# kernel-matrix-benchmarks/kernel-matrix-benchmarks

Hardware: AMD Instinct MI355X
Metric: point-pair interactions/s (N*M/s) + max |err| vs scipy, D=3 Gaussian (higher is better)
Workload: dtype f32

## Files before the change

### kernel_matrix_benchmarks_amd/csrc/kmvp_api.hip

```cpp
#include "kmvp_ctx.hpp"

namespace kmvp {

Rccl g_rccl;

namespace {
thread_local std::string g_create_error;
}

int fail(kmvp_ctx* c, int code, const std::string& msg) {
  if (c) c->err = msg;
  else g_create_error = msg;
  return code;
}
const char* create_error() { return g_create_error.c_str(); }

int ensure(kmvp_ctx* c, DevBuf& b, size_t bytes) {
  if (bytes <= b.cap && b.p) return KMVP_OK;
  if (b.p) {
    HIP_TRY(c, hipFree(b.p));
    b.p = nullptr;
    b.cap = 0;
  }
  if (bytes == 0) bytes = 16;
// ... 264 lines not shown
  if (r1 != ncclSuccess || r2 != ncclSuccess || count != world || user_rank != rank) {
    g_rccl.CommDestroy(c->comm);
    c->comm = nullptr;
    c->comm_count = 1;
    c->rank = 0;
    c->world = 1;
    return fail(c, KMVP_E_COMM, "RCCL communicator mismatch: asked for rank " + std::to_string(rank) + " of " +
                                    std::to_string(world) + " on device " + std::to_string(c->device) + ", RCCL reports rank " +
                                    std::to_string(user_rank) + " of " + std::to_string(count) + " on device " +
                                    std::to_string(dev));
  }
  c->comm_count = count;
  c->rank = rank;
  c->world = world;
  return KMVP_OK;
}

int kmvp_comm_init_host(kmvp_ctx* c, kmvp_host_allreduce_fn fn, void* user, int rank, int world) {
  if (!c || !fn || world < 1 || rank < 0 || rank >= world) return fail(c, KMVP_E_INVALID, "bad communicator arguments");
  if (c->comm) {
    g_rccl.CommDestroy(c->comm);
    c->comm = nullptr;
  }
  c->host_xchg = fn;
  c->host_user = user;
  c->comm_count = world;
  c->rank = rank;
  c->world = world;
  return KMVP_OK;
}

int kmvp_comm_world(const kmvp_ctx* c) { return (c && c->exchanges()) ? c->comm_count : 1; }
int kmvp_comm_rank(const kmvp_ctx* c) { return (c && c->exchanges()) ? c->rank : 0; }

int kmvp_set_option(kmvp_ctx* c, const char* key, int64_t value) {
  if (!c || !key) return KMVP_E_INVALID;
  const std::string k(key);
  if (k == "feed") {
    if (value < -1 || value > 1) return fail(c, KMVP_E_INVALID, "feed must be -1 (auto), 0 or 1");
    c->opt_feed = (int)value;
  } else if (k == "targets_per_lane") {
    if (value != 0 && value != 1 && value != 2 && value != 4 && value != 8)
      return fail(c, KMVP_E_INVALID, "targets_per_lane must be 0 (auto), 1, 2, 4 or 8");
    c->opt_T = (int)value;
  } else if (k == "segments") {
    if (value < 0 || value > 65535) return fail(c, KMVP_E_INVALID, "segments out of range");
    c->opt_segments = (int)value;
  } else if (k == "fast_sqdists") {
    if (value < -1 || value > 4) return fail(c, KMVP_E_INVALID, "fast_sqdists must be -1 (auto), 0, 1, 2, 3 or 4");
    c->opt_fast = (int)value;
  } else if (k == "cellmm_shape") {
    if (value < -1 || value > 1) return fail(c, KMVP_E_INVALID, "cellmm_shape must be -1 (by size), 0 (32x32x16) or 1 (16x16x32)");
    c->opt_cellmm_shape = (int)value;
  } else if (k == "cell_fused") {
    if (value < -1 || value > 1) return fail(c, KMVP_E_INVALID, "cell_fused must be -1 (automatic), 0 (two launches) or 1 (one launch where it applies)");
    c->opt_cell_fused = (int)value;
  } else if (k == "mfma_variant") {
    if (value != -1 && value != 0 && value != 1 && value != 4 && value != 5)
      return fail(c, KMVP_E_INVALID, "mfma_variant must be -1 (by kernel), 0, 1, 4 or 5");
    c->opt_mfma_variant = (int)value;
  } else if (k == "same_points_global") {
    c->opt_same_global = value != 0;
  } else if (k == "partial_shard") {
    c->opt_partial = value != 0;
  } else if (k == "fast_tiles") {
    if (value != 0 && value != 1 && value != 2 && value != 4 && value != 8)
      return fail(c, KMVP_E_INVALID, "fast_tiles must be 0 (auto), 1, 2, 4 or 8");
    c->opt_fast_tiles = (int)value;
  } else if (k == "chunk") {
    if (value < 8 || value > (1 << 24)) return fail(c, KMVP_E_INVALID, "chunk out of range");
    c->opt_chunk = (int)value;
  } else {
    return fail(c, KMVP_E_INVALID, "unknown option " + k);
  }
  return KMVP_OK;
}

int64_t kmvp_device_bytes(const kmvp_ctx* c) {
  if (!c) return 0;
  size_t t = 0;
  for (const DevBuf* b : {&c->y_raw, &c->x_raw, &c->b_raw, &c->xs, &c->rec, &c->x_scaled,
                          &c->y_scaled, &c->part, &c->partd, &c->aux, &c->sortbuf, &c->perm, &c->sums, &c->out, &c->scratch, &c->sdiag, &c->xchg, &c->kexp, &c->kshift, &c->xchgk, &c->kflag,
                    &c->sk_xs_x, &c->sk_rec_y, &c->sk_xs_y, &c->sk_rec_x, &c->sk_state,
                          &c->cell_tperm, &c->cell_sperm, &c->cell_tgrp, &c->cell_sgrp, &c->cell_slot, &c->cell_tmeta, &c->cell_sums, &c->cell_skey, &c->cell_scentre, &c->cell_scale})
    t += b->cap;
  return (int64_t)t;
}
double kmvp_last_kernel_ms(const kmvp_ctx* c) { return c ? c->last_kernel_ms : 0.0; }
double kmvp_last_total_ms(const kmvp_ctx* c) { return c ? c->last_total_ms : 0.0; }
double kmvp_last_allreduce_ms(const kmvp_ctx* c) { return c ? c->last_allreduce_ms : 0.0; }
const char* kmvp_last_kernel_name(const kmvp_ctx* c) { return c ? c->last_kernel_name : ""; }
const char* kmvp_last_dispatch_note(const kmvp_ctx* c) { return c ? c->note.c_str() : ""; }

}
```

### kernel_matrix_benchmarks_amd/csrc/kmvp_cellmm.hpp

```cpp
#pragma once
#include <hip/hip_runtime.h>
#include <stdint.h>

#include "kmvp_cell.hpp"

namespace kmvp {

#ifndef CMM_BF16
#define CMM_BF16 0
#endif
#if CMM_BF16
typedef __bf16 cmm_half;
#else
typedef _Float16 cmm_half;
#endif
typedef cmm_half f16x8 __attribute__((ext_vector_type(8)));
typedef cmm_half f16x2 __attribute__((ext_vector_type(2)));

constexpr int CMM_STAGE_TILES = 12;
constexpr int CMM_STAGE_BYTES = 8192;
constexpr int CMM_E_OFF = 0;
constexpr int CMM_B_OFF = CMM_STAGE_TILES * CELL_TILE * 16;
constexpr int CMM_HDR_OFF = CMM_B_OFF + CMM_STAGE_TILES * CELL_TILE * 4;
static_assert(CMM_HDR_OFF + CMM_STAGE_TILES * 16 <= CMM_STAGE_BYTES, "stage image too small");
constexpr float CMM_TARGET_SCALE = 64.f;
constexpr int CMM_MAX_WLOG2 = 8;

struct CellmmArgs {
  const float* xd;
  const float* tmeta;
  const unsigned char* img;
  const float* scale;
  double* part;
  int64_t n_slots;
  int64_t tile_base;
  int64_t m_stages;
  int64_t seg_stages;
  int segments;
  int tile_blocks;
};

typedef int i32x4 __attribute__((ext_vector_type(4)));

__device__ __forceinline__ f16x2 cellmm_pk(float a, float b) {
#if CMM_BF16
  f16x2 r;
  r[0] = (cmm_half)a;
  r[1] = (cmm_half)b;
  return r;
#else
  return __builtin_bit_cast(f16x2, __builtin_amdgcn_cvt_pkrtz(a, b));
#endif
}

__device__ __forceinline__ f16x8 cellmm_target_operand(const f32x4 d, int h) {
  float s[3], sh[3], sm[3];
#pragma unroll
  for (int c = 0; c < 3; ++c) {
    s[c] = d[c] * CMM_TARGET_SCALE;
    sh[c] = (float)(cmm_half)s[c];
    sm[c] = s[c] - sh[c];
  }
  const float q = CMM_TARGET_SCALE;
  float lo[8], hi[8];
  lo[0] = sh[0]; lo[1] = sh[1]; lo[2] = sh[0]; lo[3] = sh[1]; lo[4] = sm[0]; lo[5] = sm[1];
  lo[6] = d[0] * d[0] * (0.5f * q);
  lo[7] = d[1] * d[1] * (0.5f * q);
  hi[0] = sh[2]; hi[1] = d[0] * d[2] * q; hi[2] = sh[2]; hi[3] = d[0] * d[2] * q; hi[4] = sm[2];
  hi[5] = d[1] * d[2] * q;
  hi[6] = d[2] * d[2] * (0.5f * q);
  hi[7] = d[0] * d[1] * q;
  f16x8 out;
#pragma unroll
  for (int j = 0; j < 8; ++j) out[j] = (cmm_half)(h ? hi[j] : lo[j]);
  return out;
}

typedef float f32x2 __attribute__((ext_vector_type(2)));

template <int CTRL, int ROWMASK>
__device__ __forceinline__ float cellmm_dpp(float v) {
  return __int_as_float(__builtin_amdgcn_update_dpp(0, __float_as_int(v), CTRL, ROWMASK, 0xf, false));
}
__device__ __forceinline__ float cellmm_half_sum(float v) {
  v += cellmm_dpp<0x111, 0xf>(v);
  v += cellmm_dpp<0x112, 0xf>(v);
  v += cellmm_dpp<0x114, 0xf>(v);
  v += cellmm_dpp<0x118, 0xf>(v);
  v += cellmm_dpp<0x142, 0xa>(v);
  return __int_as_float(__builtin_amdgcn_readlane(__float_as_int(v), 31));
}
__device__ __forceinline__ float cellmm_cross_half_add(float v) {
// ... 144 lines not shown
      const float u1 = a14[0] * wb, u2 = a14[1] * wb;
      const f16x2 R0 = cellmm_pk(u1, u2);
      const float c1 = (float)R0[0], c2 = (float)R0[1];
      const f16x2 R1 = cellmm_pk(u1 - c1, u2 - c2);
      const f16x2 R3 = cellmm_pk(a14[2] * wb, a14[3] * wb);
      const f16x2 R2 = cellmm_pk(c1, a5 * wb);
      i32x4 yw;
      yw[0] = __builtin_bit_cast(int, R0);
      yw[1] = __builtin_bit_cast(int, R1);
      yw[2] = __builtin_bit_cast(int, R2);
      yw[3] = __builtin_bit_cast(int, R3);
      const f16x8 ya = __builtin_bit_cast(f16x8, yw);
#pragma unroll
      for (int tt = 0; tt < TT; ++tt) {
#if CMM_BF16
        acc[tt] = __builtin_amdgcn_mfma_f32_32x32x16_bf16(ya, xb[tt], acc[tt], 0, 0, 0);
#else
        acc[tt] = __builtin_amdgcn_mfma_f32_32x32x16_f16(ya, xb[tt], acc[tt], 0, 0, 0);
#endif
      }
    }
    if (s + 1 < s_end) commit(buf ^ 1);
    __syncthreads();
  }
  if (key_s >= 0) fold();

  const double inv = (double)a.scale[1];
#pragma unroll
  for (int tt = 0; tt < TT; ++tt)
    if (h == 0) a.part[(int64_t)seg * a.n_slots + (tile0 + tt - a.tile_base) * CELL_TILE + r] = outd[tt] * inv;
}


__device__ __forceinline__ float cellmm16_fold4(float a, float b, float c, float d) {
  const auto p = __builtin_amdgcn_permlane16_swap(__float_as_uint(a), __float_as_uint(b), false, false);
  const float w0 = __uint_as_float(p[0]) + __uint_as_float(p[1]);
  const auto q = __builtin_amdgcn_permlane16_swap(__float_as_uint(c), __float_as_uint(d), false, false);
  const float w1 = __uint_as_float(q[0]) + __uint_as_float(q[1]);
  const auto r = __builtin_amdgcn_permlane32_swap(__float_as_uint(w0), __float_as_uint(w1), false, false);
  return __uint_as_float(r[0]) + __uint_as_float(r[1]);
}
__device__ __forceinline__ float cellmm16_sources_sum(float v) {
  v += cellmm_dpp<0x111, 0xf>(v);
  v += cellmm_dpp<0x112, 0xf>(v);
  v += cellmm_dpp<0x114, 0xf>(v);
  v += cellmm_dpp<0x118, 0xf>(v);
  return __int_as_float(__builtin_amdgcn_readlane(__float_as_int(v), 15)) +
         __int_as_float(__builtin_amdgcn_readlane(__float_as_int(v), 47));
}

#ifndef CMM16_NOFOLD
#define CMM16_NOFOLD 0
#endif

template <int TT>
__device__ __forceinline__ void cellmm16_body(const CellmmArgs& a, int bid, unsigned char (*lds)[CMM_STAGE_BYTES]) {
  static_assert(!CMM_BF16, "f16 operands only");
  constexpr int SB = CMM_STAGE_BYTES;
  constexpr int PIECES = SB / (16 * BLOCK_THREADS);
  constexpr float LOG2E = 1.4426950408889634f;
  constexpr int HT = 2 * TT;
  constexpr int NG = (HT + 3) / 4;

  int tb, seg;
  block_to_work(bid, a.segments, a.tile_blocks, tb, seg);
  const int lane = threadIdx.x & 63;
  const int wave = threadIdx.x >> 6;
  const int cc = lane & 15;
  const int kg = lane >> 4;
  const int h = kg & 1;
  const int rs = 16 * (kg >> 1) + cc;
  const int64_t tile0 = a.tile_base + ((int64_t)tb * WAVES_PER_BLOCK + wave) * TT;

  float cT[3];
  f16x8 xb[HT];
#pragma unroll
  for (int u = 0; u < HT; ++u) {
    const f32x4 v = *reinterpret_cast<const f32x4*>(a.xd + ((tile0 + (u >> 1)) * CELL_TILE + 16 * (u & 1) + cc) * 4);
    xb[u] = cellmm_target_operand(v, h);
  }
  {
    const f32x4 m = *reinterpret_cast<const f32x4*>(a.tmeta + tile0 * 4);
#pragma unroll
    for (int c = 0; c < 3; ++c) cT[c] = __int_as_float(__builtin_amdgcn_readfirstlane(__float_as_int(m[c])));
  }
  float dl[NG][3], U[NG], vprev[NG];
  double outd[NG];
#pragma unroll
  for (int g = 0; g < NG; ++g) {
    const int u = 4 * g + kg < HT ? 4 * g + kg : HT - 1;
    const f32x4 v = *reinterpret_cast<const f32x4*>(a.xd + ((tile0 + (u >> 1)) * CELL_TILE + 16 * (u & 1) + cc) * 4);
#pragma unroll
    for (int c = 0; c < 3; ++c) dl[g][c] = v[c];
    U[g] = 0.f;
    vprev[g] = 0.f;
    outd[g] = 0.0;
  }

  f32x4 acc[HT];
#pragma unroll
  for (int u = 0; u < HT; ++u)
#pragma unroll
    for (int k = 0; k < 4; ++k) acc[u][k] = 0.f;

  const int64_t s_begin = (int64_t)seg * a.seg_stages;
  int64_t s_end = s_begin + a.seg_stages;
  if (s_end > a.m_stages) s_end = a.m_stages;

  f32x4 pre[PIECES];
  auto fetch = [&](int64_t s) {
    const unsigned char* src = a.img + s * SB;
#pragma unroll
    for (int p = 0; p < PIECES; ++p)
      pre[p] = *reinterpret_cast<const f32x4*>(src + (p * BLOCK_THREADS + (int)threadIdx.x) * 16);
  };
  auto commit = [&](int buf) {
#pragma unroll
    for (int p = 0; p < PIECES; ++p)
      *reinterpret_cast<f32x4*>(&lds[buf][(p * BLOCK_THREADS + (int)threadIdx.x) * 16]) = pre[p];
  };
  if (s_begin < s_end) {
    fetch(s_begin);
    commit(0);
  }
  __syncthreads();

  int key_s = -2;
  float S0 = 0.f, S0c = 0.f;
  float D1[3] = {0.f, 0.f, 0.f};

  auto fold = [&]() {
#if CMM16_NOFOLD
    asm volatile("" ::"v"(S0), "v"(S0c));
#else
    const float s0 = cellmm16_sources_sum(S0) * CMM_TARGET_SCALE;
    float x[4 * NG];
#pragma unroll
    for (int u = 0; u < 4 * NG; ++u) x[u] = u < HT ? (acc[u][0] + acc[u][1]) + (acc[u][2] + acc[u][3]) : 0.f;
#pragma unroll
    for (int g = 0; g < NG; ++g) {
      const float v = cellmm16_fold4(x[4 * g], x[4 * g + 1], x[4 * g + 2], x[4 * g + 3]);
      outd[g] += (double)(U[g] * ((v - vprev[g]) + s0));
      vprev[g] = v;
    }
#endif
    S0 = 0.f;
    S0c = 0.f;
  };
  auto new_cell = [&](const f32x4 cs, int ks) {
    if (key_s >= 0) fold();
    key_s = ks;
#pragma unroll
    for (int c = 0; c < 3; ++c) D1[c] = (cT[c] - cs[c]) * LOG2E;
#if !CMM16_NOFOLD
#pragma unroll
    for (int g = 0; g < NG; ++g) {
      float s2 = 0.f;
#pragma unroll
      for (int c = 0; c < 3; ++c) {
        const float df = dl[g][c] + (cT[c] - cs[c]);
        s2 = fmaf(df, df, s2);
      }
      U[g] = kexp2(s2 * -LOG2E);
    }
#endif
  };

  for (int64_t s = s_begin; s < s_end; ++s) {
    const int buf = (int)((s - s_begin) & 1);
    if (s + 1 < s_end) fetch(s + 1);
    const unsigned char* base = &lds[buf][0];
    const unsigned char* p_ef = base + CMM_E_OFF + rs * 16;
    const unsigned char* p_b = base + CMM_B_OFF + rs * 4;
    const f32x4* hdr = reinterpret_cast<const f32x4*>(base + CMM_HDR_OFF);
    const int keys = lane < CMM_STAGE_TILES ? __float_as_int(hdr[lane < CMM_STAGE_TILES ? lane : 0][3]) : -1;
#pragma unroll 1
    for (int q = 0; q < CMM_STAGE_TILES; ++q) {
      const int ks = __builtin_amdgcn_readlane(keys, q);
      if (ks < 0) break;
      if (ks != key_s) new_cell(hdr[q], ks);
      const f32x4 ef = *reinterpret_cast<const f32x4*>(p_ef);
      const float bq = *reinterpret_cast<const float*>(p_b);
      p_ef += CELL_TILE * 16;
      p_b += CELL_TILE * 4;
      const float m0 = h ? ef[2] : ef[0];
      const float m1 = h ? ef[0] : ef[1];
      const float m2 = h ? ef[2] : 1.f;
      const f32x4 a14 = f32x4{m0, m1 * m2, m0 * m0, m1 * ef[1]};
      const float a5 = ef[1] * m2;
      const float arg = fmaf(ef[0], D1[0], fmaf(ef[1], D1[1], fmaf(ef[2], D1[2], ef[3])));
      const float wb = kexp2(arg) * bq;
      {
        const float yk = wb - S0c;
        const float tk = S0 + yk;
        S0c = (tk - S0) - yk;
        S0 = tk;
      }
      const float u1 = a14[0] * wb, u2 = a14[1] * wb;
      const f16x2 R0 = cellmm_pk(u1, u2);
      const float c1 = (float)R0[0], c2 = (float)R0[1];
      const f16x2 R1 = cellmm_pk(u1 - c1, u2 - c2);
      const f16x2 R3 = cellmm_pk(a14[2] * wb, a14[3] * wb);
      const f16x2 R2 = cellmm_pk(c1, a5 * wb);
      i32x4 yw;
      yw[0] = __builtin_bit_cast(int, R0);
      yw[1] = __builtin_bit_cast(int, R1);
      yw[2] = __builtin_bit_cast(int, R2);
      yw[3] = __builtin_bit_cast(int, R3);
      const f16x8 ya = __builtin_bit_cast(f16x8, yw);
#pragma unroll
      for (int u = 0; u < HT; ++u) acc[u] = __builtin_amdgcn_mfma_f32_16x16x32_f16(ya, xb[u], acc[u], 0, 0, 0);
    }
    if (s + 1 < s_end) commit(buf ^ 1);
    __syncthreads();
  }
  if (key_s >= 0) fold();
#if CMM16_NOFOLD
#pragma unroll
  for (int u = 0; u < HT; ++u) asm volatile("" ::"v"(acc[u][0]), "v"(acc[u][1]), "v"(acc[u][2]), "v"(acc[u][3]));
#endif

  const double inv = (double)a.scale[1];
#pragma unroll
  for (int g = 0; g < NG; ++g)
    if (4 * g + kg < HT)
      a.part[(int64_t)seg * a.n_slots + (tile0 + 2 * g + (kg >> 1) - a.tile_base) * CELL_TILE + 16 * h + cc] = outd[g] * inv;
}

template <int TT>
__global__ void __launch_bounds__(BLOCK_THREADS) __attribute__((amdgpu_waves_per_eu(TT >= 8 ? 2 : 1)))
cellmm16_kernel(const CellmmArgs a, const CellmmArgs rest, const int main_grid) {
  __shared__ __attribute__((aligned(16))) unsigned char lds[2][CMM_STAGE_BYTES];
  if constexpr (TT > CELL_REST_TT) {
    const FusedCellWork w = fused_cell_work((int64_t)blockIdx.x, (int64_t)main_grid);
    if (w.list) {
      cellmm16_body<CELL_REST_TT>(rest, (int)w.local, lds);
      return;
    }
  }
  cellmm16_body<TT>(a, (int)blockIdx.x, lds);
}

hipError_t launch_cellmm_gaussian(int TT, int shape, const CellmmArgs& args, dim3 grid, hipStream_t stream, const char** kernel_name);
hipError_t launch_cellmm16_fused(int TT, const CellmmArgs& main, const CellmmArgs& rest, int64_t main_grid, int64_t rest_grid,
                                 hipStream_t stream, const char** kernel_name);

}
```

### kernel_matrix_benchmarks_amd/csrc/kmvp_ctx.hpp

```cpp
#pragma once
#include <dlfcn.h>
#include <hip/hip_runtime.h>
#include <rccl/rccl.h>
#include <stdint.h>
#include <stdlib.h>
#include <string.h>

#include <algorithm>
#include <cmath>
#include <string>
#include <vector>

#include "../../include/kmvp.h"
#include "kmvp_internal.hpp"

namespace kmvp {

enum : int { LAYOUT_LOWD = 0, LAYOUT_FAST = 1, LAYOUT_MFMA = 2, LAYOUT_CFAST = 3, LAYOUT_CELL = 4, LAYOUT_CELL64 = 5, LAYOUT_CELLMM = 6, LAYOUT_FASTMM = 7, LAYOUT_CFASTMM = 8 };

struct DevBuf {
  void* p = nullptr;
  size_t cap = 0;
};

// ... 50 lines not shown
      error = "librccl lacks an expected symbol";
      return false;
    }
    return true;
  }
};extern Rccl g_rccl;

}

struct kmvp_ctx {
  using DevBuf = kmvp::DevBuf;
  int device = 0;
  hipStream_t stream = nullptr;
  hipEvent_t ev[5] = {nullptr, nullptr, nullptr, nullptr, nullptr};
  std::string err;

  int dtype = -1;
  int D = 0, E = 0;
  int64_t M = 0, N = 0, j_offset = 0, m_total = 0;
  bool same_points = false;
  bool have_points = false, have_signal = false, density = false;
  bool async_product = false;
  bool diag_on = false;
  int64_t diag_n = 0;
  double diag_ridge = 0.0, diag_min = 0.0;

  DevBuf y_raw, x_raw, b_raw;
  DevBuf xs, rec;
  DevBuf partd;
  DevBuf aux;
  DevBuf sortbuf, perm;
  DevBuf x_scaled, y_scaled;
  DevBuf cell_tperm, cell_sperm, cell_tgrp, cell_sgrp, cell_slot, cell_tmeta, cell_sums, cell_skey, cell_scentre, cell_scale;
  DevBuf part, sums, out;
  DevBuf xchg;
  DevBuf kexp, kshift, xchgk;
  DevBuf kflag;
  DevBuf scratch;
  DevBuf sdiag;
  DevBuf sk_xs_x, sk_rec_y, sk_xs_y, sk_rec_x, sk_state;
  uint64_t sk_points_ver = 0;
  uint64_t points_ver = 0, signal_ver = 0;
  int packed_layout = -1;
  int packed_kernel = -1, packed_sig = -1, packed_T = -1;
  uint64_t packed_points_ver = 0, packed_signal_ver = 0;
  int gen_kernel = -1;
  uint64_t gen_points_ver = 0;
  int64_t out_n = 0;
  int out_e = 0;

  int opt_feed = -1, opt_T = 0, opt_segments = 0, opt_chunk = 512;
  int opt_fast = -1, opt_fast_tiles = 0;
  int opt_cellmm_shape = -1;
  int opt_cell_fused = -1;
  int opt_mfma_variant = -1;
  int opt_same_global = 0;
  int opt_partial = 0;
  uint64_t perm_ver = 0;
  uint64_t cell_ver = 0;
  int cell_state = 0;
  int cell_tt = 0, cell_tt_req = 0;
  float cell_lo[3] = {0.f, 0.f, 0.f}, cell_hh[3] = {1.f, 1.f, 1.f};
  int cell_g[3] = {1, 1, 1};
  int64_t cell_n_tiles = 0, cell_m_tiles = 0;
  int64_t cell_n_main = 0, cell_n_rest = 0;
  float cloud_radius2 = INFINITY;
  uint64_t centre_ver = 0;

  ncclComm_t comm = nullptr;
  int rank = 0, world = 1;
  kmvp_host_allreduce_fn host_xchg = nullptr;
  void* host_user = nullptr;
  std::vector<double> host_buf;
  bool exchanges() const { return comm != nullptr || host_xchg != nullptr; }

  int comm_count = 1;
  float last_kernel_ms = 0.f, last_total_ms = 0.f, last_allreduce_ms = 0.f;
  const char* last_kernel_name = "";
  std::string note;
};

namespace kmvp {

int fail(kmvp_ctx* c, int code, const std::string& msg);
const char* create_error();

#define HIP_TRY(c, expr)                                                                     \
  do {                                                                                       \
    hipError_t e_ = (expr);                                                                  \
    if (e_ != hipSuccess)                                                                    \
      return kmvp::fail((c), e_ == hipErrorOutOfMemory ? KMVP_E_NOMEM : KMVP_E_DEVICE,       \
                        std::string(#expr) + ": " + hipGetErrorString(e_));                  \
  } while (0)

inline size_t elem_size(int dtype) { return dtype == KMVP_F64 ? 8 : 4; }
inline unsigned blocks_for(int64_t n, int threads = 256) { return (unsigned)((n + threads - 1) / threads); }

int ensure(kmvp_ctx* c, DevBuf& b, size_t bytes);
void release(DevBuf& b);

int run_product(kmvp_ctx* c, int kernel, bool normalise);
int measure_clouds(kmvp_ctx* c, int dtype, int64_t M, int64_t N, int D);
int prepare_points(kmvp_ctx* c, int kernel);
int run_gradient(kmvp_ctx* c, int kernel);
int run_logsumexp(kmvp_ctx* c, int kernel);
int run_logsumexp_grad(kmvp_ctx* c, int kernel);

int cg_solve(kmvp_ctx* c, int kernel, const void* a_host, int E, double rtol, int maxit, double* out_b,
             int* iters, double* resid);
int minres_solve(kmvp_ctx* c, int kernel, const void* a_host, int E, double rtol, int maxit,
                 double* out_b, int* iters, double* resid);

int sinkhorn_solve(kmvp_ctx* c, int kernel, const double* log_a, const double* log_b, double tol, int maxit, double* u,
                   double* v, int* iters, double* err);

}
```

### kernel_matrix_benchmarks_amd/csrc/kmvp_plan.hpp

```cpp
#pragma once
#include <algorithm>
#include <cstdint>
#include <vector>

namespace kmvp {

constexpr int WAVES_PER_BLOCK = 4;
constexpr int CELL_TILE = 32;
constexpr int CELL_REST_TT = 2;
constexpr int STAGED_TILE = 32;
constexpr int64_t SMALL_PROBLEM_TARGETS = 32768;
constexpr int SEG_SPLIT_FROM = 16;
constexpr int64_t MAX_GRID = 0x7fffffff;

inline int64_t round_up(int64_t v, int64_t q) { return (v + q - 1) / q * q; }
inline bool small_problem(int64_t N) { return N < SMALL_PROBLEM_TARGETS; }


struct SegmentRule {
  int64_t stage_bytes;
  int cols;
  int64_t min_seg = 1;
  bool small = false;
  int64_t l2_seg_bytes = 2 << 20;
// ... 145 lines not shown
  int64_t grid(int r) const { return blocks[r] * segments[r]; }
  size_t region_offset(int cols, int r) const { return r ? (size_t)segments[0] * cols * slots[0] : 0; }
  size_t part_doubles(int cols) const { return ((size_t)segments[0] * slots[0] + (size_t)segments[1] * slots[1]) * cols; }
};

inline CellSplit cell_split(int64_t N, int64_t m_tiles, int64_t n_main, int64_t n_rest, int tt, int opt_segments,
                            int stage_tiles, SegmentRule main) {
  CellSplit s;
  main.small = small_problem(N);
  if (main.small) main.min_seg = 1;
  s.m_stages = (m_tiles + stage_tiles - 1) / stage_tiles;
  s.n_slots = (n_main + n_rest) * CELL_TILE;
  s.blocks[0] = n_main / (tt * WAVES_PER_BLOCK);
  s.blocks[1] = n_rest / (CELL_REST_TT * WAVES_PER_BLOCK);
  s.slots[0] = n_main * CELL_TILE;
  s.slots[1] = n_rest * CELL_TILE;
  s.segments[0] = stage_segments(opt_segments, std::max<int64_t>(1, s.blocks[0]), s.m_stages, s.n_slots, main);
  s.seg_stages[0] = (s.m_stages + s.segments[0] - 1) / s.segments[0];
  s.segments[1] = 0;
  s.seg_stages[1] = 1;
  if (s.blocks[1] > 0) {
    SegmentRule rest = main;
    rest.min_seg = 1;
    rest.target_blocks = 1536;
    const int seg = choose_segments(opt_segments, s.blocks[1], s.m_stages, s.n_slots, rest);
    s.seg_stages[1] = (s.m_stages + seg - 1) / seg;
    s.segments[1] = (int)((s.m_stages + s.seg_stages[1] - 1) / s.seg_stages[1]);
  }
  return s;
}


struct FusedCellWork {
  int list;
  int64_t local;
};
constexpr FusedCellWork fused_cell_work(int64_t bid, int64_t main_grid) {
  return bid < main_grid ? FusedCellWork{0, bid} : FusedCellWork{1, bid - main_grid};
}

struct FusedCellGrid {
  bool fused;
  int64_t main_grid, rest_grid, total;
};
inline FusedCellGrid fused_cell_grid(const CellSplit& s, int tt, int opt_fused) {
  FusedCellGrid g;
  g.main_grid = s.grid(0);
  g.rest_grid = s.grid(1);
  g.total = g.main_grid + g.rest_grid;
  g.fused = opt_fused != 0 && tt > CELL_REST_TT && s.blocks[1] > 0 && g.total <= MAX_GRID;
  return g;
}

}
```

### kernel_matrix_benchmarks_amd/csrc/kmvp_product.hip

```cpp
#include "kmvp_ctx.hpp"
#include <vector>
#include "kmvp_cell_pack.hpp"
#include "kmvp_cell64_pack.hpp"
#include "kmvp_cellmm_pack.hpp"
#include "kmvp_cfast_pack.hpp"
#include "kmvp_fast_pack.hpp"
#include "kmvp_fastmm_pack.hpp"
#include "kmvp_cfastmm_pack.hpp"
#include "kmvp_mfma_pack.hpp"

namespace kmvp {
namespace {

template <typename real>
hipError_t launch_lowd(int kernel, int D, int E, int sig, LowdTuning tune,
                       const LowdArgs<real>& args, dim3 grid, hipStream_t s, const char** name);
template <>
hipError_t launch_lowd<float>(int kernel, int D, int E, int sig, LowdTuning tune,
                              const LowdArgs<float>& args, dim3 grid, hipStream_t s,
                              const char** name) {
  switch (kernel) {
    case K_GAUSSIAN: return launch_lowd_gaussian_f32(D, E, sig, tune, args, grid, s, name);
    case K_ABSEXP: return launch_lowd_absexp_f32(D, E, sig, tune, args, grid, s, name);
    case K_INVDIST: return launch_lowd_invdist_f32(D, E, sig, tune, args, grid, s, name);
// ... 1208 lines not shown
    }
  }
  return true;
}
void cell_store_grid(kmvp_ctx* c, const CellGrid& grid) {
  for (int a = 0; a < 3; ++a) {
    c->cell_lo[a] = grid.lo[a];
    c->cell_g[a] = grid.g[a];
    c->cell_hh[a] = grid.h[a];
  }
}
void cell_load_grid(const kmvp_ctx* c, CellGrid& grid) {
  for (int a = 0; a < 3; ++a) {
    grid.lo[a] = c->cell_lo[a];
    grid.g[a] = c->cell_g[a];
    grid.h[a] = c->cell_hh[a];
    grid.inv_h[a] = 1.f / c->cell_hh[a];
  }
}

inline double cell_ps_per_tile(int TT) { return TT >= 8 ? CMM_PS_PER_TILE_MAIN : (TT >= 4 ? CMM_PS_PER_TILE_TT4 : CMM_PS_PER_TILE_REST); }

int cell_prepare(kmvp_ctx* c, int TT) {
  if (c->cell_ver == c->points_ver && c->cell_state != 0 && (c->cell_state < 0 || c->cell_tt_req == TT)) return KMVP_OK;
  c->cell_tt_req = TT;
  c->cell_ver = c->points_ver;
  c->cell_state = -1;
  const int D = c->D;
  if (D > CELL_MAX_D || !(c->cloud_radius2 < INFINITY) || c->N > 0x3fffffff || c->M > 0x3fffffff) return KMVP_OK;
  float aux[FAST_AUX_FLOATS];
  HIP_TRY(c, hipMemcpyAsync(aux, c->aux.p, sizeof(aux), hipMemcpyDeviceToHost, c->stream));
  HIP_TRY(c, hipStreamSynchronize(c->stream));
  CellGrid grid;
  if (!cell_make_grid(aux, D, (float)(std::sqrt(2.f * CELL_T_MAX / (float)D)), grid)) return KMVP_OK;
  int rc;
  std::vector<unsigned> keys;
  if ((rc = cell_sort(c, c->y_raw.p, c->M, grid, c->cell_sperm, keys))) return rc;
  const TileList sources = cell_tiles(keys.data(), c->M);
  if ((rc = upload_tiles(c, sources, c->cell_sgrp))) return rc;
  c->cell_m_tiles = (int64_t)sources.size();
  if (!c->same_points && (rc = cell_sort(c, c->x_raw.p, c->N, grid, c->cell_tperm, keys))) return rc;
  if (TT == 0) {
    double best = INFINITY;
    for (int t : {8, 4, 2}) {
      int64_t nm, nr;
      cell_split_count(keys.data(), (int64_t)keys.size(), t, &nm, &nr);
      const double cost = cell_ps_per_tile(t) * (double)nm + cell_ps_per_tile(2) * (double)nr;
      if (cost < best) {
        best = cost;
        TT = t;
      }
    }
  }
  if ((rc = upload_tiles(c, cell_tiles_split(keys.data(), (int64_t)keys.size(), TT, &c->cell_n_main, &c->cell_n_rest), c->cell_tgrp)))
    return rc;
  c->cell_n_tiles = c->cell_n_main + c->cell_n_rest;
  c->cell_tt = TT;
  cell_store_grid(c, grid);
  c->cell_state = 1;
  c->packed_layout = -1;
  return KMVP_OK;
}

double cell_padding(const kmvp_ctx* c) {
  const double t = (double)c->cell_n_tiles * CELL_TILE / (double)std::max<int64_t>(c->N, 1);
  const double s = (double)c->cell_m_tiles * CELL_TILE / (double)std::max<int64_t>(c->M, 1);
  return std::max(t, s);
}

CellSplit cell_plan(const kmvp_ctx* c, int stage_tiles, SegmentRule main) {
  return cell_split(c->N, c->cell_m_tiles, c->cell_n_main, c->cell_n_rest, c->cell_tt, c->opt_segments, stage_tiles, main);
}
double* cell_region(const kmvp_ctx* c, const CellSplit& s, int cols, int r) { return (double*)c->part.p + s.region_offset(cols, r); }
template <class Args>
void cell_args(const kmvp_ctx* c, const CellSplit& s, int cols, int r, Args& a) {
  a.part = cell_region(c, s, cols, r);
  a.n_slots = s.slots[r];
  a.tile_base = r ? c->cell_n_main : 0;
  a.seg_stages = s.seg_stages[r];
  a.segments = s.segments[r];
  a.tile_blocks = (int)s.blocks[r];
}
inline int cell_tt(const kmvp_ctx* c, int r) { return r ? CELL_REST_TT : c->cell_tt; }

int pack_cell_targets(kmvp_ctx* c, const CellGrid& grid) {
  const int64_t n_tiles = c->cell_n_tiles;
  const float* x_raw = (const float*)(c->same_points ? c->y_raw.p : c->x_raw.p);
  const int* tperm = (const int*)(c->same_points ? c->cell_sperm.p : c->cell_tperm.p);
  const int* tgrp = (const int*)c->cell_tgrp.p;
  int rc;
  if ((rc = ensure(c, c->xs, (size_t)n_tiles * CELL_TILE * 4 * sizeof(float)))) return rc;
  if ((rc = ensure(c, c->cell_tmeta, (size_t)n_tiles * 4 * sizeof(float)))) return rc;
  if ((rc = ensure(c, c->cell_slot, (size_t)c->N * sizeof(int)))) return rc;
  hipLaunchKernelGGL(pack_cell_targets_kernel, dim3((unsigned)n_tiles), dim3(CELL_TILE), 0, c->stream, x_raw, tperm,
                     tgrp, tgrp + n_tiles, (const unsigned*)(tgrp + 2 * n_tiles), n_tiles, c->D,
                     grid, (float*)c->xs.p, (float*)c->cell_tmeta.p, (int*)c->cell_slot.p);
  return KMVP_OK;
}


int run_product_cell(kmvp_ctx* c, int sig) {
  const int D = c->D;
  const int E = 1;
  const int NE = sig == SIG_NORM ? 2 : 1;
  const int64_t N = c->N;
  SegmentRule rule(CELL_STAGE_BYTES, NE);
  rule.min_seg = 4;
  const CellSplit s = cell_plan(c, CELL_STAGE_TILES, rule);
// ... 51 lines not shown

int cellmm_wlog2(const kmvp_ctx* c) {
  double arg = 0.0;
  for (int a = 0; a < c->D; ++a) arg += (double)c->cell_hh[a] * ((double)c->cell_g[a] * c->cell_hh[a]);
  return (int)std::ceil(arg * 1.4426950408889634);
}

int run_product_cellmm(kmvp_ctx* c, int sig) {
  const int D = c->D;
  const int E = sig == SIG_DENSITY ? 1 : c->E;
  const int NE = sig == SIG_NORM ? E + 1 : E;
  const int64_t N = c->N;
  const int TT = c->cell_tt;
  SegmentRule rule(CMM_STAGE_BYTES, 1);
  rule.min_seg = 2;
  rule.l2_seg_bytes = 3 << 20;
  rule.target_blocks = 7168;
  const CellSplit s = cell_plan(c, CMM_STAGE_TILES, rule);
  const int64_t m_stages = s.m_stages, n_slots = s.n_slots;
  int rc;
  CellGrid grid;
  cell_load_grid(c, grid);

  const PackKey key = {LAYOUT_CELLMM, K_GAUSSIAN, TT};
  const int image_sig = NE > 1 ? -1 : sig;
  const bool sig_stale = signal_stale(c, key, image_sig);
  const int* sgrp = (const int*)c->cell_sgrp.p;
  if ((rc = ensure(c, c->cell_scale, 64))) return rc;
  float* scale = (float*)c->cell_scale.p;
  unsigned* bmax = (unsigned*)c->cell_scale.p + 4;
  HIP_TRY(c, mark(c, 0));
  if (points_stale(c, key)) {
    if ((rc = pack_cell_targets(c, grid))) return rc;
    if ((rc = ensure(c, c->rec, (size_t)m_stages * CMM_STAGE_BYTES))) return rc;
    hipLaunchKernelGGL(pack_cellmm_points_kernel, dim3((unsigned)(m_stages * CMM_STAGE_TILES)), dim3(CELL_TILE), 0,
                       c->stream, (const float*)c->y_raw.p, (const int*)c->cell_sperm.p, sgrp, sgrp + c->cell_m_tiles,
                       (const unsigned*)(sgrp + 2 * c->cell_m_tiles), c->cell_m_tiles, D, grid, (unsigned char*)c->rec.p);
    HIP_TRY(c, hipGetLastError());
  }
  record_packed(c, key, image_sig);

  if ((rc = ensure(c, c->part, s.part_doubles(1) * sizeof(double)))) return rc;
  if ((rc = ensure(c, c->sums, (size_t)NE * N * sizeof(double)))) return rc;
  if ((rc = ensure(c, c->cell_sums, (size_t)NE * n_slots * sizeof(double)))) return rc;
  const int shape = c->opt_cellmm_shape >= 0 ? c->opt_cellmm_shape : ((TT >= 8 && c->N >= 500000 && c->M >= 100000) ? 1 : 0);
  FusedCellGrid fg = fused_cell_grid(s, TT, c->opt_cell_fused);
  if (shape != 1) fg.fused = false;
  CellmmArgs a;
  a.xd = (const float*)c->xs.p;
  a.tmeta = (const float*)c->cell_tmeta.p;
  a.img = (const unsigned char*)c->rec.p;
  a.scale = scale;
  a.m_stages = m_stages;
  if (NE == 1 && !sig_stale) HIP_TRY(c, mark(c, 0));
  for (int col = 0; col < NE; ++col) {
    if (sig_stale) {
      const float* b = (sig == SIG_DENSITY || col == E) ? (const float*)nullptr : (const float*)c->b_raw.p;
      HIP_TRY(c, hipMemsetAsync(bmax, 0, sizeof(unsigned), c->stream));
      if (b)
        hipLaunchKernelGGL(cellmm_absmax_kernel, dim3((unsigned)std::min<int64_t>(1024, (c->M + 255) / 256)), dim3(256), 0,
                           c->stream, b, c->M, E, col, bmax);
      hipLaunchKernelGGL(cellmm_scale_kernel, dim3(1), dim3(1), 0, c->stream, (const unsigned*)bmax, cellmm_wlog2(c),
                         b ? 0 : 1, scale);
      hipLaunchKernelGGL(pack_cellmm_signal_kernel, dim3((unsigned)(m_stages * CMM_STAGE_TILES)), dim3(CELL_TILE), 0,
                         c->stream, b, E, col, (const int*)c->cell_sperm.p, sgrp, sgrp + c->cell_m_tiles, c->cell_m_tiles,
                         (const float*)scale, (unsigned char*)c->rec.p);
      HIP_TRY(c, hipGetLastError());
      if (NE == 1) HIP_TRY(c, mark(c, 0));
    }
    hipError_t le = hipSuccess;
    if (fg.fused) {
      CellmmArgs ar = a;
      cell_args(c, s, 1, 0, a);
      cell_args(c, s, 1, 1, ar);
      le = launch_cellmm16_fused(TT, a, ar, fg.main_grid, fg.rest_grid, c->stream, &c->last_kernel_name);
    } else {
      for (int r = 0; r < 2 && le == hipSuccess; ++r)
        if (s.blocks[r] > 0) {
          cell_args(c, s, 1, r, a);
          le = launch_cellmm_gaussian(cell_tt(c, r), shape, a, dim3((unsigned)s.grid(r)), c->stream, &c->last_kernel_name);
        }
    }
    if (le == hipErrorInvalidValue) return fail(c, KMVP_E_UNSUPPORTED, "fast_tiles must be 1, 2, 4 or 8");
    HIP_TRY(c, le);
    if (NE == 1) HIP_TRY(c, mark(c, 1));
    double* col_sums = (double*)c->cell_sums.p + (size_t)col * n_slots;
    for (int r = 0; r < 2; ++r)
      if (s.blocks[r] > 0)
        hipLaunchKernelGGL(reduce_segments_kernel, dim3(blocks_for(s.slots[r])), dim3(256), 0, c->stream,
                           (const double*)cell_region(c, s, 1, r), col_sums + (r ? s.slots[0] : 0), s.slots[r], s.segments[r], 0);
    HIP_TRY(c, hipGetLastError());
  }
  if (NE > 1) HIP_TRY(c, mark(c, 1));

  hipLaunchKernelGGL(gather_cells_kernel, dim3(blocks_for((int64_t)NE * N)), dim3(256), 0, c->stream,
                     (const double*)c->cell_sums.p, (const int*)c->cell_slot.p, (double*)c->sums.p, N, n_slots, NE);
  HIP_TRY(c, hipGetLastError());
  return finish_product(c, (int64_t)NE * N, N, N, E, sig);
}


int cell64_prepare(kmvp_ctx* c) {
  if (c->cell_ver == c->points_ver && c->cell_state != 0) return KMVP_OK;
  c->cell_ver = c->points_ver;
  c->cell_state = -1;
  const int D = c->D;
  if (D > CELL_MAX_D || !(c->cloud_radius2 < INFINITY) || c->N > 0x3fffffff || c->M > 0x3fffffff) return KMVP_OK;
  float aux[FAST_AUX_FLOATS];
  HIP_TRY(c, hipMemcpyAsync(aux, c->aux.p, sizeof(aux), hipMemcpyDeviceToHost, c->stream));
  HIP_TRY(c, hipStreamSynchronize(c->stream));
  CellGrid grid;
  if (!cell_make_grid(aux, D, (float)((float)std::sqrt(2.0 * CELL64_T_MAX / (double)D)), grid)) return KMVP_OK;
  int rc;
  std::vector<unsigned> keys;
  if ((rc = cell_sort(c, c->y_raw.p, c->M, grid, c->cell_sperm, keys, &c->cell_skey))) return rc;
  std::vector<int> runs;
  std::vector<double> centres;
  for_each_key_run(keys.data(), c->M, [&](int64_t first, int64_t count, unsigned key) {
    runs.push_back((int)first);
    runs.push_back((int)count);
    for (int a = 0; a < 3; ++a) centres.push_back(a < D ? cell64_centre(key, a, grid) : 0.0);
    centres.push_back(0.0);
  });
  c->cell_m_tiles = (int64_t)runs.size() / 2;
  if ((rc = ensure(c, c->cell_sgrp, runs.size() * sizeof(int)))) return rc;
  if ((rc = ensure(c, c->cell_scentre, centres.size() * sizeof(double)))) return rc;
  HIP_TRY(c, hipMemcpyAsync(c->cell_sgrp.p, runs.data(), runs.size() * sizeof(int), hipMemcpyHostToDevice, c->stream));
  HIP_TRY(c, hipMemcpyAsync(c->cell_scentre.p, centres.data(), centres.size() * sizeof(double), hipMemcpyHostToDevice, c->stream));
  HIP_TRY(c, hipStreamSynchronize(c->stream));
  if (!c->same_points && (rc = cell_sort(c, c->x_raw.p, c->N, grid, c->cell_tperm, keys))) return rc;
  const TileList targets = cell_tiles(keys.data(), (int64_t)keys.size(), CELL64_TILE);
  if ((rc = upload_tiles(c, targets, c->cell_tgrp))) return rc;
  c->cell_n_tiles = (int64_t)targets.size();
  c->cell_tt = 1;
  cell_store_grid(c, grid);
  c->cell_state = 1;
  c->packed_layout = -1;
  return KMVP_OK;
}

int run_product_cell64(kmvp_ctx* c, int sig) {
  const int D = c->D;
  const int NE = sig == SIG_NORM ? 2 : 1;
  const int64_t N = c->N, M = c->M;
  const int64_t n_tiles = round_up(c->cell_n_tiles, WAVES_PER_BLOCK);
  const int64_t n_slots = n_tiles * CELL64_TILE;
// ... 559 lines not shown
```

Baseline: 40750 billion.

## Share source-operand construction across waves when a workgroup's targets lie in one cell

When all four wavefronts of a workgroup handle target tiles in the same cell, the exp-weighted f16 source operands no longer depend on the wave. Each wave now builds a quarter of the stage's operands once into a second LDS buffer, and all waves read them for their MFMAs. This removes redundant exp2 and packing work per wave. In exchange it adds LDS traffic, a second LDS array, and a two-stage-ahead prefetch. A host-side count of eligible workgroups is added for reporting, and a runtime option controls the path.

```diff
diff --git a/kernel_matrix_benchmarks_amd/csrc/kmvp_api.hip b/kernel_matrix_benchmarks_amd/csrc/kmvp_api.hip
--- a/kernel_matrix_benchmarks_amd/csrc/kmvp_api.hip
+++ b/kernel_matrix_benchmarks_amd/csrc/kmvp_api.hip
@@ -340,6 +340,9 @@
   } else if (k == "cellmm_shape") {
     if (value < -1 || value > 1) return fail(c, KMVP_E_INVALID, "cellmm_shape must be -1 (by size), 0 (32x32x16) or 1 (16x16x32)");
     c->opt_cellmm_shape = (int)value;
+  } else if (k == "cell_shared") {
+    if (value < -1 || value > 1) return fail(c, KMVP_E_INVALID, "cell_shared must be -1 (automatic), 0 (never) or 1 (the shared body where it applies)");
+    c->opt_cell_shared = (int)value;
   } else if (k == "cell_fused") {
     if (value < -1 || value > 1) return fail(c, KMVP_E_INVALID, "cell_fused must be -1 (automatic), 0 (two launches) or 1 (one launch where it applies)");
     c->opt_cell_fused = (int)value;
diff --git a/kernel_matrix_benchmarks_amd/csrc/kmvp_cellmm.hpp b/kernel_matrix_benchmarks_amd/csrc/kmvp_cellmm.hpp
--- a/kernel_matrix_benchmarks_amd/csrc/kmvp_cellmm.hpp
+++ b/kernel_matrix_benchmarks_amd/csrc/kmvp_cellmm.hpp
@@ -38,6 +38,7 @@
   int64_t seg_stages;
   int segments;
   int tile_blocks;
+  int shared;
 };
 
 typedef int i32x4 __attribute__((ext_vector_type(4)));
@@ -288,9 +289,59 @@
 #ifndef CMM16_NOFOLD
 #define CMM16_NOFOLD 0
 #endif
-
-template <int TT>
-__device__ __forceinline__ void cellmm16_body(const CellmmArgs& a, int bid, unsigned char (*lds)[CMM_STAGE_BYTES]) {
+#ifndef CMM16_NOBUILD
+#define CMM16_NOBUILD 0
+#endif
+
+struct Cmm16Operand {
+  f16x8 ya;
+  float w, bq;
+};
+__device__ __forceinline__ void cellmm16_kahan(const Cmm16Operand& o, float& S0, float& S0c) {
+  const float yk = fmaf(o.bq, o.w, -S0c);
+  const float tk = S0 + yk;
+  S0c = (tk - S0) - yk;
+  S0 = tk;
+}
+__device__ __forceinline__ Cmm16Operand cellmm16_operand(const f32x4 ef, const float bq, const float (&D1)[3], const int h) {
+#if CMM16_NOBUILD == 1
+  return {__builtin_bit_cast(f16x8, ef), 1.f, bq};
+#elif CMM16_NOBUILD == 3
+  const i32x4 fin = __builtin_bit_cast(i32x4, ef) & (int)0xbfffbfff;
+  return {__builtin_bit_cast(f16x8, fin), 1.f, bq};
+#else
+  const float m0 = h ? ef[2] : ef[0];
+  const float m1 = h ? ef[0] : ef[1];
+  const float m2 = h ? ef[2] : 1.f;
+  const f32x4 a14 = f32x4{m0, m1 * m2, m0 * m0, m1 * ef[1]};
+  const float a5 = ef[1] * m2;
+  const float arg = fmaf(ef[0], D1[0], fmaf(ef[1], D1[1], fmaf(ef[2], D1[2], ef[3])));
+  const float w = kexp2(arg);
+  const float wb = w * bq;
+  const float u1 = a14[0] * wb, u2 = a14[1] * wb;
+  const f16x2 R0 = cellmm_pk(u1, u2);
+  const float c1 = (float)R0[0], c2 = (float)R0[1];
+  const f16x2 R1 = cellmm_pk(u1 - c1, u2 - c2);
+  const f16x2 R3 = cellmm_pk(a14[2] * wb, a14[3] * wb);
+  const f16x2 R2 = cellmm_pk(c1, a5 * wb);
+  i32x4 yw;
+  yw[0] = __builtin_bit_cast(int, R0);
+  yw[1] = __builtin_bit_cast(int, R1);
+  yw[2] = __builtin_bit_cast(int, R2);
+  yw[3] = __builtin_bit_cast(int, R3);
+  return {__builtin_bit_cast(f16x8, yw), w, bq};
+#endif
+}
+
+constexpr int CMM_OP_YA_OFF = 0;
+constexpr int CMM_OP_WB_OFF = CMM_STAGE_TILES * 64 * 16;
+constexpr int CMM_OP_HDR_OFF = CMM_OP_WB_OFF + CMM_STAGE_TILES * CELL_TILE * 8;
+constexpr int CMM_OP_STAGE_BYTES = CMM_OP_HDR_OFF + CMM_STAGE_TILES * 16;
+static_assert(CMM_OP_STAGE_BYTES % 16 == 0 && CMM_STAGE_TILES % WAVES_PER_BLOCK == 0, "operand stage layout");
+
+template <int TT, bool SHARED>
+__device__ __forceinline__ void cellmm16_body(const CellmmArgs& a, int bid, unsigned char (*lds)[CMM_STAGE_BYTES],
+                                              unsigned char (*ops)[CMM_OP_STAGE_BYTES]) {
   static_assert(!CMM_BF16, "f16 operands only");
   constexpr int SB = CMM_STAGE_BYTES;
   constexpr int PIECES = SB / (16 * BLOCK_THREADS);
@@ -301,7 +352,7 @@
   int tb, seg;
   block_to_work(bid, a.segments, a.tile_blocks, tb, seg);
   const int lane = threadIdx.x & 63;
-  const int wave = threadIdx.x >> 6;
+  const int wave = SHARED ? __builtin_amdgcn_readfirstlane(threadIdx.x >> 6) : threadIdx.x >> 6;
   const int cc = lane & 15;
   const int kg = lane >> 4;
   const int h = kg & 1;
@@ -355,7 +406,44 @@
     for (int p = 0; p < PIECES; ++p)
       *reinterpret_cast<f32x4*>(&lds[buf][(p * BLOCK_THREADS + (int)threadIdx.x) * 16]) = pre[p];
   };
-  if (s_begin < s_end) {
+  auto build = [&](int buf) {
+    const unsigned char* raw = &lds[buf][0];
+    unsigned char* op = &ops[buf][0];
+    constexpr int NB = CMM_STAGE_TILES / WAVES_PER_BLOCK;
+    f32x4 csq[NB], efq[NB];
+    float bqq[NB];
+#pragma unroll
+    for (int j = 0; j < NB; ++j) {
+      const int q = wave * NB + j;
+      csq[j] = reinterpret_cast<const f32x4*>(raw + CMM_HDR_OFF)[q];
+      efq[j] = *reinterpret_cast<const f32x4*>(raw + CMM_E_OFF + (q * CELL_TILE + rs) * 16);
+      bqq[j] = *reinterpret_cast<const float*>(raw + CMM_B_OFF + (q * CELL_TILE + rs) * 4);
+    }
+#pragma unroll
+    for (int j = 0; j < NB; ++j) {
+      const int q = wave * NB + j;
+      const f32x4 cs = csq[j];
+      float D1q[3];
+#pragma unroll
+      for (int c = 0; c < 3; ++c) D1q[c] = (cT[c] - cs[c]) * LOG2E;
+      const Cmm16Operand o = cellmm16_operand(efq[j], bqq[j], D1q, h);
+      *reinterpret_cast<f16x8*>(op + CMM_OP_YA_OFF + (q * 64 + lane) * 16) = o.ya;
+      *reinterpret_cast<f32x2*>(op + CMM_OP_WB_OFF + (q * CELL_TILE + rs) * 8) = f32x2{o.w, o.bq};
+      if (lane == 0) *reinterpret_cast<f32x4*>(op + CMM_OP_HDR_OFF + q * 16) = cs;
+    }
+  };
+  if constexpr (SHARED) {
+    if (s_begin < s_end) {
+      fetch(s_begin);
+      commit(0);
+    }
+    if (s_begin + 1 < s_end) {
+      fetch(s_begin + 1);
+      commit(1);
+    }
+    __syncthreads();
+    if (s_begin < s_end) build(0);
+  } else if (s_begin < s_end) {
     fetch(s_begin);
     commit(0);
   }
@@ -386,8 +474,10 @@
   auto new_cell = [&](const f32x4 cs, int ks) {
     if (key_s >= 0) fold();
     key_s = ks;
-#pragma unroll
-    for (int c = 0; c < 3; ++c) D1[c] = (cT[c] - cs[c]) * LOG2E;
+    if constexpr (!SHARED) {
+#pragma unroll
+      for (int c = 0; c < 3; ++c) D1[c] = (cT[c] - cs[c]) * LOG2E;
+    }
 #if !CMM16_NOFOLD
 #pragma unroll
     for (int g = 0; g < NG; ++g) {
@@ -404,50 +494,46 @@
 
   for (int64_t s = s_begin; s < s_end; ++s) {
     const int buf = (int)((s - s_begin) & 1);
-    if (s + 1 < s_end) fetch(s + 1);
-    const unsigned char* base = &lds[buf][0];
-    const unsigned char* p_ef = base + CMM_E_OFF + rs * 16;
-    const unsigned char* p_b = base + CMM_B_OFF + rs * 4;
-    const f32x4* hdr = reinterpret_cast<const f32x4*>(base + CMM_HDR_OFF);
+    constexpr int AHEAD = SHARED ? 2 : 1;
+    if (s + AHEAD < s_end) fetch(s + AHEAD);
+    if constexpr (SHARED) {
+      if (s + 1 < s_end) build(buf ^ 1);
+    }
+    const unsigned char* base = SHARED ? &ops[buf][0] : &lds[buf][0];
+    const unsigned char* p_ef = SHARED ? base + CMM_OP_YA_OFF + lane * 16 : base + CMM_E_OFF + rs * 16;
+    const unsigned char* p_b = SHARED ? base + CMM_OP_WB_OFF + rs * 8 : base + CMM_B_OFF + rs * 4;
+    const f32x4* hdr = reinterpret_cast<const f32x4*>(base + (SHARED ? CMM_OP_HDR_OFF : CMM_HDR_OFF));
     const int keys = lane < CMM_STAGE_TILES ? __float_as_int(hdr[lane < CMM_STAGE_TILES ? lane : 0][3]) : -1;
+#if CMM16_NOBUILD == 2
+    Cmm16Operand o_first = {};
+#endif
 #pragma unroll 1
     for (int q = 0; q < CMM_STAGE_TILES; ++q) {
       const int ks = __builtin_amdgcn_readlane(keys, q);
       if (ks < 0) break;
       if (ks != key_s) new_cell(hdr[q], ks);
       const f32x4 ef = *reinterpret_cast<const f32x4*>(p_ef);
-      const float bq = *reinterpret_cast<const float*>(p_b);
-      p_ef += CELL_TILE * 16;
-      p_b += CELL_TILE * 4;
-      const float m0 = h ? ef[2] : ef[0];
-      const float m1 = h ? ef[0] : ef[1];
-      const float m2 = h ? ef[2] : 1.f;
-      const f32x4 a14 = f32x4{m0, m1 * m2, m0 * m0, m1 * ef[1]};
-      const float a5 = ef[1] * m2;
-      const float arg = fmaf(ef[0], D1[0], fmaf(ef[1], D1[1], fmaf(ef[2], D1[2], ef[3])));
-      const float wb = kexp2(arg) * bq;
-      {
-        const float yk = wb - S0c;
-        const float tk = S0 + yk;
-        S0c = (tk - S0) - yk;
-        S0 = tk;
+      Cmm16Operand o;
+      if constexpr (SHARED) {
+        const f32x2 wb = *reinterpret_cast<const f32x2*>(p_b);
+        o = {__builtin_bit_cast(f16x8, ef), wb[0], wb[1]};
+      } else {
+        const float bq = *reinterpret_cast<const float*>(p_b);
+#if CMM16_NOBUILD == 2
+        if (q == 0) o_first = cellmm16_operand(ef, bq, D1, h);
+        else asm volatile("" ::"v"(ef), "v"(bq));
+        o = o_first;
+#else
+        o = cellmm16_operand(ef, bq, D1, h);
+#endif
       }
-      const float u1 = a14[0] * wb, u2 = a14[1] * wb;
-      const f16x2 R0 = cellmm_pk(u1, u2);
-      const float c1 = (float)R0[0], c2 = (float)R0[1];
-      const f16x2 R1 = cellmm_pk(u1 - c1, u2 - c2);
-      const f16x2 R3 = cellmm_pk(a14[2] * wb, a14[3] * wb);
-      const f16x2 R2 = cellmm_pk(c1, a5 * wb);
-      i32x4 yw;
-      yw[0] = __builtin_bit_cast(int, R0);
-      yw[1] = __builtin_bit_cast(int, R1);
-      yw[2] = __builtin_bit_cast(int, R2);
-      yw[3] = __builtin_bit_cast(int, R3);
-      const f16x8 ya = __builtin_bit_cast(f16x8, yw);
-#pragma unroll
-      for (int u = 0; u < HT; ++u) acc[u] = __builtin_amdgcn_mfma_f32_16x16x32_f16(ya, xb[u], acc[u], 0, 0, 0);
-    }
-    if (s + 1 < s_end) commit(buf ^ 1);
+      p_ef += SHARED ? 64 * 16 : CELL_TILE * 16;
+      p_b += SHARED ? CELL_TILE * 8 : CELL_TILE * 4;
+      cellmm16_kahan(o, S0, S0c);
+#pragma unroll
+      for (int u = 0; u < HT; ++u) acc[u] = __builtin_amdgcn_mfma_f32_16x16x32_f16(o.ya, xb[u], acc[u], 0, 0, 0);
+    }
+    if (s + AHEAD < s_end) commit(SHARED ? buf : buf ^ 1);
     __syncthreads();
   }
   if (key_s >= 0) fold();
@@ -468,13 +554,24 @@
 cellmm16_kernel(const CellmmArgs a, const CellmmArgs rest, const int main_grid) {
   __shared__ __attribute__((aligned(16))) unsigned char lds[2][CMM_STAGE_BYTES];
   if constexpr (TT > CELL_REST_TT) {
+    __shared__ __attribute__((aligned(16))) unsigned char ops[2][CMM_OP_STAGE_BYTES];
     const FusedCellWork w = fused_cell_work((int64_t)blockIdx.x, (int64_t)main_grid);
     if (w.list) {
-      cellmm16_body<CELL_REST_TT>(rest, (int)w.local, lds);
+      cellmm16_body<CELL_REST_TT, false>(rest, (int)w.local, lds, nullptr);
       return;
     }
-  }
-  cellmm16_body<TT>(a, (int)blockIdx.x, lds);
+    if (a.shared && !CMM16_NOBUILD) {
+      int tb, seg;
+      block_to_work((int)blockIdx.x, a.segments, a.tile_blocks, tb, seg);
+      const unsigned* tkey = reinterpret_cast<const unsigned*>(a.tmeta) + 3;
+      const int64_t t0 = a.tile_base + (int64_t)tb * WAVES_PER_BLOCK * TT;
+      if (one_cell_block(tkey[t0 * 4], tkey[(t0 + TT) * 4], tkey[(t0 + 2 * TT) * 4], tkey[(t0 + 3 * TT) * 4])) {
+        cellmm16_body<TT, true>(a, (int)blockIdx.x, lds, ops);
+        return;
+      }
+    }
+  }
+  cellmm16_body<TT, false>(a, (int)blockIdx.x, lds, nullptr);
 }
 
 hipError_t launch_cellmm_gaussian(int TT, int shape, const CellmmArgs& args, dim3 grid, hipStream_t stream, const char** kernel_name);
diff --git a/kernel_matrix_benchmarks_amd/csrc/kmvp_ctx.hpp b/kernel_matrix_benchmarks_amd/csrc/kmvp_ctx.hpp
--- a/kernel_matrix_benchmarks_amd/csrc/kmvp_ctx.hpp
+++ b/kernel_matrix_benchmarks_amd/csrc/kmvp_ctx.hpp
@@ -126,6 +126,7 @@
   int opt_feed = -1, opt_T = 0, opt_segments = 0, opt_chunk = 512;
   int opt_fast = -1, opt_fast_tiles = 0;
   int opt_cellmm_shape = -1;
+  int opt_cell_shared = -1;
   int opt_cell_fused = -1;
   int opt_mfma_variant = -1;
   int opt_same_global = 0;
@@ -137,6 +138,7 @@
   float cell_lo[3] = {0.f, 0.f, 0.f}, cell_hh[3] = {1.f, 1.f, 1.f};
   int cell_g[3] = {1, 1, 1};
   int64_t cell_n_tiles = 0, cell_m_tiles = 0;
+  int64_t cell_one_cell_blocks = 0;
   int64_t cell_n_main = 0, cell_n_rest = 0;
   float cloud_radius2 = INFINITY;
   uint64_t centre_ver = 0;
diff --git a/kernel_matrix_benchmarks_amd/csrc/kmvp_plan.hpp b/kernel_matrix_benchmarks_amd/csrc/kmvp_plan.hpp
--- a/kernel_matrix_benchmarks_amd/csrc/kmvp_plan.hpp
+++ b/kernel_matrix_benchmarks_amd/csrc/kmvp_plan.hpp
@@ -221,4 +221,19 @@
   return g;
 }
 
-}
+
+constexpr unsigned CELL_EMPTY_TILE_BIT = 1u << 30;
+constexpr bool one_cell_block(unsigned k0, unsigned k1, unsigned k2, unsigned k3) {
+  return (((k0 ^ k1) | (k0 ^ k2) | (k0 ^ k3)) & ~CELL_EMPTY_TILE_BIT) == 0;
+}
+static_assert(WAVES_PER_BLOCK == 4, "one_cell_block compares four wavefronts");
+
+inline bool cell_shared_applies(int tt, int opt_shared) { return opt_shared != 0 && tt > CELL_REST_TT; }
+inline int64_t count_one_cell_blocks(const unsigned* main_keys, int64_t n_main, int tt) {
+  int64_t n = 0;
+  for (int64_t t = 0; t + (int64_t)WAVES_PER_BLOCK * tt <= n_main; t += (int64_t)WAVES_PER_BLOCK * tt)
+    n += one_cell_block(main_keys[t], main_keys[t + tt], main_keys[t + 2 * tt], main_keys[t + 3 * tt]) ? 1 : 0;
+  return n;
+}
+
+}
diff --git a/kernel_matrix_benchmarks_amd/csrc/kmvp_product.hip b/kernel_matrix_benchmarks_amd/csrc/kmvp_product.hip
--- a/kernel_matrix_benchmarks_amd/csrc/kmvp_product.hip
+++ b/kernel_matrix_benchmarks_amd/csrc/kmvp_product.hip
@@ -1284,8 +1284,9 @@
       }
     }
   }
-  if ((rc = upload_tiles(c, cell_tiles_split(keys.data(), (int64_t)keys.size(), TT, &c->cell_n_main, &c->cell_n_rest), c->cell_tgrp)))
-    return rc;
+  const TileList targets = cell_tiles_split(keys.data(), (int64_t)keys.size(), TT, &c->cell_n_main, &c->cell_n_rest);
+  if ((rc = upload_tiles(c, targets, c->cell_tgrp))) return rc;
+  c->cell_one_cell_blocks = count_one_cell_blocks(targets.key.data(), c->cell_n_main, TT);
   c->cell_n_tiles = c->cell_n_main + c->cell_n_rest;
   c->cell_tt = TT;
   cell_store_grid(c, grid);
@@ -1443,6 +1444,7 @@
   a.img = (const unsigned char*)c->rec.p;
   a.scale = scale;
   a.m_stages = m_stages;
+  a.shared = shape == 1 && cell_shared_applies(TT, c->opt_cell_shared) ? 1 : 0;
   if (NE == 1 && !sig_stale) HIP_TRY(c, mark(c, 0));
   for (int col = 0; col < NE; ++col) {
     if (sig_stale) {
@@ -1483,6 +1485,12 @@
     HIP_TRY(c, hipGetLastError());
   }
   if (NE > 1) HIP_TRY(c, mark(c, 1));
+  if (shape == 1 && s.blocks[0] > 0) {
+    char buf[128];
+    snprintf(buf, sizeof(buf), "%scellmm16 shared body: %lld of %lld MAIN workgroups", c->note.empty() ? "" : "; ",
+             (long long)(a.shared ? c->cell_one_cell_blocks * s.segments[0] : 0), (long long)s.grid(0));
+    c->note += buf;
+  }
 
   hipLaunchKernelGGL(gather_cells_kernel, dim3(blocks_for((int64_t)NE * N)), dim3(256), 0, c->stream,
                      (const double*)c->cell_sums.p, (const int*)c->cell_slot.p, (double*)c->sums.p, N, n_slots, NE);
```

Result: no change. 40940 billion (median of 6 runs) (+0.5%).
